# tomershay100/mp3-steganography-lib

Hardware: AMD Instinct MI355X
Metric: MP3 frames/sec (decode+re-encode) @44.1kHz stereo 128kbps, 1→8 GPU (higher is better)
Workload: dtype f64 (decode) / int32 (encode); 1 GPU; 10000-frame full decode->stego-embed->re-encode pipeline per MI355X (BASELINE configs[2]); MP3 main data + side info resident in HBM, MP3 frames out; the message cursor chain is decided and the serial chains of the rate loop are checked on the device inside every step; frames_per_gpu=10000, channels=2, message_bits=536, chain_verdict_units_to_redo=0, message_variant_entries=1874, parallelism=frames sharded over 1 GPU(s), no collective

## Files before the change

### mp3-steganography-lib_amd/csrc/k_encode.hpp

```cpp
#pragma once
#include <type_traits>
#include "analysis_plan.h"

namespace mp3s {

__device__ __forceinline__ int32_t mulhi_vs(int32_t v, int32_t s)
{
    int32_t r;
    asm("v_mul_hi_i32 %0, %1, %2" : "=v"(r) : "v"(v), "s"(s));
    return r;
}
typedef int32_t i32x4 __attribute__((ext_vector_type(4)));
typedef int32_t i32x16 __attribute__((ext_vector_type(16)));
typedef int32_t i32x8 __attribute__((ext_vector_type(8)));
template <int B, int E, class F>
__device__ __forceinline__ void static_for(F &&f)
{
    if constexpr (B < E) { f(std::integral_constant<int, B>{}); static_for<B + 1, E>(f); }
}

constexpr int ENC_ROW = 34;
constexpr int ENC_LDS_DW = 79 * 17 + 1;

constexpr int ENC_TROW = 33;
template <bool TILE, class Between>
__device__ __forceinline__ void enc_analysis_wave(const int16_t *__restrict__ pcm, const mp3s_frame_hdr *__restrict__ hdr, long Ts, int ch, long t0, int lane,
                                                  uint32_t *lds, int32_t *__restrict__ SB, uint32_t *rows, long tile_t0, long lo, long hi, Between between)
{
    int16_t *tw = reinterpret_cast<int16_t *>(lds);
    if ((reinterpret_cast<uintptr_t>(pcm) & 15u) == 0) {
        const int c0 = (int)(t0 - 15) * 8, c1 = (int)Ts * 8;
        const uint4 *gp = reinterpret_cast<const uint4 *>(pcm);
        const uint32_t sel = ch ? 0x07060302u : 0x05040100u;
        for (int c = lane; c < 79 * 8; c += 64) {
            const int gc = c0 + c;
            uint4 q = make_uint4(0, 0, 0, 0);
            if (gc >= 0 && gc < c1) q = gp[gc];
            uint2 o;
            o.x = __builtin_amdgcn_perm(q.y, q.x, sel);
            o.y = __builtin_amdgcn_perm(q.w, q.z, sel);
            uint32_t *dst = reinterpret_cast<uint32_t *>(tw + (c >> 3) * ENC_ROW + (c & 7) * 4);
            dst[0] = o.x; dst[1] = o.y;
        }
    } else {
        for (int e = lane; e < 79 * 32; e += 64) {
            const int r = e >> 5, s = e & 31;
            const long row = t0 - 15 + r;
            int16_t v = 0;
            if (row >= 0 && row < Ts) v = pcm[(row * 32 + s) * 2 + ch];
            tw[r * ENC_ROW + s] = v;
        }
    }
    __builtin_amdgcn_s_waitcnt(0xc07f);
    __builtin_amdgcn_wave_barrier();
    const long t = t0 + lane;
    const bool valid = t >= 0 && t < Ts;
    long s0 = 0;
    if (valid) s0 = (long)hdr[t / 36].stream_first * 36;

    int32_t y[64];
    const bool starts_inside = __ballot(valid && (t - 15) < s0) != 0;
    const uint32_t tw_lds = (uint32_t)(uintptr_t)(__attribute__((address_space(3))) const int16_t *)tw;
    uint32_t xs[16];
#pragma unroll
    for (int i = 0; i < 16; i++) xs[i] = 0;
#define MP3S_LDS_HI16(reg, addr, off) asm volatile("ds_read_u16_d16_hi %0, %1 offset:%2" : "+v"(reg) : "v"(addr), "n"(off))
    auto window_sums = [&](auto masked) {
    auto trip = [&](int k, auto first) {
        const i32x16 *ewa = reinterpret_cast<const i32x16 *>(c_tab.enwindow + 64 * k), *ewb = ewa + 4;
#pragma unroll
        for (int h = 0; h < 2; h++) {
            const i32x16 a0 = ewa[2 * h], a1 = ewa[2 * h + 1];
            const i32x16 b0 = ewb[2 * h], b1 = ewb[2 * h + 1];
            const int back_a = 2 * k + h, back_b = back_a + 2;
            const bool in_a = (t - back_a) >= s0, in_b = (t - back_b) >= s0;
            const uint32_t ra = tw_lds + (uint32_t)((lane + 15 - back_a) * ENC_ROW * 2), rb = ra - 2 * ENC_ROW * 2;
#pragma unroll
            for (int cb = 0; cb < 4; cb++) {
#pragma unroll
                for (int e = 0; e < 8; e++) {
                    MP3S_LDS_HI16(xs[e], ra, (cb * 8 + e) * 2);
                    MP3S_LDS_HI16(xs[8 + e], rb, (cb * 8 + e) * 2);
                }
                asm volatile("s_waitcnt lgkmcnt(0)" : "+v"(xs[0]), "+v"(xs[1]), "+v"(xs[2]), "+v"(xs[3]), "+v"(xs[4]), "+v"(xs[5]), "+v"(xs[6]), "+v"(xs[7]),
                             "+v"(xs[8]), "+v"(xs[9]), "+v"(xs[10]), "+v"(xs[11]), "+v"(xs[12]), "+v"(xs[13]), "+v"(xs[14]), "+v"(xs[15]));
#pragma unroll
                for (int e = 0; e < 8; e++) {
                    const int col = cb * 8 + e, c = 31 - col;
                    int32_t xa = (int32_t)xs[e], xb = (int32_t)xs[8 + e];
                    if (decltype(masked)::value && !in_a) xa = 0;
                    if (decltype(masked)::value && !in_b) xb = 0;
                    const int32_t two = mulhi_vs(xa, c < 16 ? a0[c & 15] : a1[c & 15]) + mulhi_vs(xb, c < 16 ? b0[c & 15] : b1[c & 15]);
                    if (decltype(first)::value) y[h * 32 + c] = two; else y[h * 32 + c] += two;
                }
                __builtin_amdgcn_sched_barrier(0);
            }
        }
    };
    trip(0, std::true_type{});
#pragma unroll 1
    for (int k = 2; k < 8; k += 2) trip(k, std::false_type{});
    };
    if (starts_inside) window_sums(std::true_type{}); else window_sums(std::false_type{});
#undef MP3S_LDS_HI16
    const bool odd_slot = (t & 1) != 0;
    __builtin_amdgcn_wave_barrier();
    between();
    uint32_t *ot = lds;
    uint32_t *out = TILE ? nullptr : reinterpret_cast<uint32_t *>(SB) + ((long)ch * Ts + t0) * 32;
    const int n_rows = (Ts - t0) < 64 ? (int)(Ts - t0) : 64;
    uint32_t *trow = TILE ? rows + (valid && t >= lo && t < hi ? (t - tile_t0) : -1) * ENC_TROW : nullptr;
    int32_t a[4] = {0, 0, 0, 0};
    i32x8 cur[4], nxt[4];
    typedef const int32_t __attribute__((address_space(4))) *fl_ptr;
    fl_ptr flp = (fl_ptr)&c_tab.fl[0][0];
    asm volatile("" : "+s"(flp));
    auto load_block = [&](auto nc, i32x8 (&c)[4]) {
        constexpr int N = decltype(nc)::value, P = N >> 3, B = N & 7;
        constexpr int O[4] = {P, 15 - P, 16 + P, 31 - P};
#pragma unroll
        for (int o = 0; o < 4; o++) c[o] = *(const i32x8 __attribute__((address_space(4))) *)(flp + O[o] * 64 + 8 * B);
    };
    load_block(std::integral_constant<int, 0>{}, cur);
    static_for<0, 64>([&](auto nc) {
        constexpr int N = decltype(nc)::value, P = N >> 3, B = N & 7;
        __builtin_amdgcn_sched_barrier(0);
        __builtin_amdgcn_s_waitcnt(0xc07f);
        __builtin_amdgcn_sched_barrier(0);
        if constexpr (N < 63) load_block(std::integral_constant<int, N + 1>{}, nxt);
        __builtin_amdgcn_sched_barrier(0);
#pragma unroll
        for (int j = 0; j < 8; j += 2) {
            int32_t m[2][4];
#pragma unroll
            for (int e = 0; e < 2; e++) {
                const int k = B * 8 + j + e;
                const unsigned plan = ANALYSIS_PLAN[P][k];
                const int32_t cj[4] = {cur[0][j + e], cur[1][j + e], cur[2][j + e], cur[3][j + e]};
#pragma unroll
                for (int o = 0; o < 4; o++) {
                    const unsigned rep = (plan >> (2 * o)) & 3u;
                    if ((plan >> (8 + o)) & 1u) m[e][o] = 0;
                    else if (rep == (unsigned)o) m[e][o] = mulhi_vs(y[k], cj[o]);
                    else m[e][o] = m[e][rep];
                }
            }
#pragma unroll
            for (int o = 0; o < 4; o++) {
                a[o] += m[0][o] + m[1][o];
                asm("" : "+v"(a[o]));
            }
            if (j == 2) __builtin_amdgcn_sched_barrier(0);
        }
        if constexpr (B == 7) {
            if (odd_slot) {
                if (P & 1) { a[0] = (int32_t)(0u - (uint32_t)a[0]); a[2] = (int32_t)(0u - (uint32_t)a[2]); }
                else       { a[1] = (int32_t)(0u - (uint32_t)a[1]); a[3] = (int32_t)(0u - (uint32_t)a[3]); }
            }
            constexpr int q = P & 3;
            if constexpr (TILE) {
                trow[P] = (uint32_t)a[0]; trow[15 - P] = (uint32_t)a[1]; trow[16 + P] = (uint32_t)a[2]; trow[31 - P] = (uint32_t)a[3];
            } else {
            ot[lane * 17 + q] = (uint32_t)a[0];
            ot[lane * 17 + 4 + 3 - q] = (uint32_t)a[1];
            ot[lane * 17 + 8 + q] = (uint32_t)a[2];
            ot[lane * 17 + 12 + 3 - q] = (uint32_t)a[3];
            }
            a[0] = a[1] = a[2] = a[3] = 0;
            if constexpr (q == 3 && !TILE) {
                constexpr int g = P >> 2;
                __builtin_amdgcn_s_waitcnt(0xc07f);
                __builtin_amdgcn_wave_barrier();
                const int piece = lane & 3;
#pragma unroll
                for (int r = lane >> 2; r < 64; r += 16) {
                    const uint32_t *src = ot + r * 17 + piece * 4;
                    const uint4 v = make_uint4(src[0], src[1], src[2], src[3]);
                    if (r < n_rows) *reinterpret_cast<uint4 *>(out + r * 32 + g * 16 + piece * 4) = v;
                }
                __builtin_amdgcn_s_waitcnt(0xc07f);
                __builtin_amdgcn_wave_barrier();
            }
        }
        if constexpr (N < 63) {
#pragma unroll
            for (int o = 0; o < 4; o++) cur[o] = nxt[o];
        }
    });
}

__device__ __forceinline__ int sb_pos(int band) { return (int)((0x37621540u >> (4 * (band >> 2))) & 7u) * 4 + (band & 3); }
__global__ __launch_bounds__(256, 5) void k_enc_analysis(
    const int16_t *__restrict__ pcm, const mp3s_frame_hdr *__restrict__ hdr, int n_frames,
    int32_t *__restrict__ SB, long Ts)
{
    __shared__ __attribute__((aligned(16))) uint32_t lds_all[4][ENC_LDS_DW];
    static_assert(79 * ENC_ROW * 2 <= ENC_LDS_DW * 4, "PCM tile must fit");
    const int wave = __builtin_amdgcn_readfirstlane(threadIdx.x >> 6), lane = threadIdx.x & 63;
    const long wid = (long)xcd_tile() * 4 + wave;
    const int ch = (int)(wid & 1);
    const long t0 = (wid >> 1) * 64;
    if (t0 >= Ts) return;
    enc_analysis_wave<false>(pcm, hdr, Ts, ch, t0, lane, lds_all[wave], SB, nullptr, 0, 0, 0, [] {});
}

constexpr int MD_ROW = 33, MD_BLK = 18 * MD_ROW;

__device__ __forceinline__ void enc_mdct_pair(const int32_t (&in)[54], int32_t *xs, int lane, int32_t *__restrict__ mdct, long ga, long g_lo, long g_hi)
{
    const int ch = lane >> 5, band = lane & 31;
    int32_t *x0 = xs + ch * MD_BLK + band, *x1 = x0 + 2 * MD_BLK;
    struct Coef { i32x4 q[9]; };
    auto load_coef = [&](int k) {
        Coef c;
        const i32x4 *crow = reinterpret_cast<const i32x4 *>(c_tab.cos_l[k]);
#pragma unroll
        for (int q = 0; q < 9; q++) c.q[q] = crow[q];
        return c;
    };
    Coef cur = load_coef(0);
#pragma unroll 2
    for (int k = 0; k < 18; k++) {
        asm volatile("" ::"s"(cur.q[0].x));
        __builtin_amdgcn_sched_barrier(0);
        const Coef nxt = load_coef(k < 17 ? k + 1 : 17);
        __builtin_amdgcn_sched_barrier(0);
        int32_t a0 = 0, a1 = 0;
#pragma unroll
        for (int q = 0; q < 9; q++) {
            const i32x4 c = cur.q[q];
            a0 += mulhi_vs(in[4 * q], c.x);     a1 += mulhi_vs(in[18 + 4 * q], c.x);
            a0 += mulhi_vs(in[4 * q + 1], c.y); a1 += mulhi_vs(in[19 + 4 * q], c.y);
            a0 += mulhi_vs(in[4 * q + 2], c.z); a1 += mulhi_vs(in[20 + 4 * q], c.z);
            a0 += mulhi_vs(in[4 * q + 3], c.w); a1 += mulhi_vs(in[21 + 4 * q], c.w);
        }
        x0[k * MD_ROW] = a0;
        x1[k * MD_ROW] = a1;
        __builtin_amdgcn_sched_barrier(0);
        cur = nxt;
    }
    __builtin_amdgcn_s_waitcnt(0xc07f);
    __builtin_amdgcn_wave_barrier();
    if (band >= 1) {
#pragma unroll
        for (int g = 0; g < 2; g++)
#pragma unroll
            for (int i = 0; i < 8; i++) {
                int32_t *pa = x0 + g * 2 * MD_BLK + i * MD_ROW, *pb = x0 + g * 2 * MD_BLK + (17 - i) * MD_ROW - 1;
                const int64_t cs = c_tab.mdct_cs[i], ca = c_tab.mdct_ca[i];
                const int64_t a = *pa, b = *pb;
                *pa = (int32_t)((a * cs - b * ca) >> 31);
                *pb = (int32_t)((a * ca + b * cs) >> 31);
            }
    }
    __builtin_amdgcn_s_waitcnt(0xc07f);
    __builtin_amdgcn_wave_barrier();
#pragma unroll
    for (int q = 0; q < 4; q++) {
        const long g = ga + (q >> 1);
        if (g < g_lo || g >= g_hi) continue;
        const int32_t *src = xs + q * MD_BLK;
        int32_t *o = mdct + (((g >> 1) * 2 + (q & 1)) * 2 + (g & 1)) * 576;
#pragma unroll
        for (int t = 0; t < 9; t++) {
            const int e = lane + 64 * t, b = (e * 3641) >> 16, k = e - 18 * b;
            o[e] = src[k * MD_ROW + b];
        }
    }
}

__global__ __launch_bounds__(256, 4) void k_enc_mdct(
    const int32_t *__restrict__ SB, long Ts, const mp3s_frame_hdr *__restrict__ hdr, int n_frames,
    int32_t *__restrict__ mdct)
{
    __shared__ int32_t xs_all[4][4 * MD_BLK];
    const int wave = __builtin_amdgcn_readfirstlane(threadIdx.x >> 6), lane = threadIdx.x & 63;
    const int f = xcd_tile() * 4 + wave;
    if (f >= n_frames) return;
    const int ch = lane >> 5, band = lane & 31;
    const bool has_prev = f > (int)hdr[f].stream_first;
    const int32_t *row = SB + ((long)ch * Ts + (long)f * 36) * 32 + sb_pos(band);
    const int32_t *prow = has_prev ? row - 18 * 32 : row;
    int32_t in[54];
#pragma unroll
    for (int j = 0; j < 18; j++) {
        const int32_t pv = prow[j * 32];
        in[j] = has_prev ? pv : 0;
        in[18 + j] = row[j * 32];
        in[36 + j] = row[(18 + j) * 32];
    }
    enc_mdct_pair(in, xs_all[wave], lane, mdct, 2l * f, 2l * f, 2l * f + 2);
}

constexpr int EF_GR = 13, EF_SLOTS = 18 * (EF_GR + 1), EF_WAVES = 8;
constexpr int EF_TILE_DW = 2 * (EF_SLOTS + 1) * ENC_TROW;
static_assert(EF_SLOTS <= 4 * 64, "four analysis waves per channel");
static_assert(EF_WAVES * ENC_LDS_DW <= EF_TILE_DW, "the waves' PCM staging fits the tile");
static_assert(((EF_GR + 1) / 2) * 4 * MD_BLK <= EF_TILE_DW, "the MDCT waves' butterfly tiles fit the tile");

__global__ __launch_bounds__(EF_WAVES * 64, 4) void k_enc_fused(
    const int16_t *__restrict__ pcm, const mp3s_frame_hdr *__restrict__ hdr, int n_frames, int32_t *__restrict__ mdct)
{
    __shared__ __attribute__((aligned(16))) uint32_t tile[EF_TILE_DW];
    const int wave = __builtin_amdgcn_readfirstlane(threadIdx.x >> 6), lane = threadIdx.x & 63;
    const long Ts = (long)n_frames * 36, n_gran = (long)n_frames * 2;
    const long g0 = (long)xcd_tile() * EF_GR;
    const long s0 = g0 * 18, t_first = s0 - 18;
    {
        const int ch = wave >> 2;
        const long t0 = t_first + 64 * (wave & 3);
        uint32_t *rows = tile + ((long)ch * (EF_SLOTS + 1) + 1) * ENC_TROW;
        enc_analysis_wave<true>(pcm, hdr, Ts, ch, t0, lane, tile + wave * ENC_LDS_DW, nullptr, rows, t_first, t_first, t_first + EF_SLOTS,
                                [] { __syncthreads(); });
    }
    __syncthreads();
    const long ga = g0 - (g0 & 1) + 2 * wave;
    const long g_hi = g0 + EF_GR < n_gran ? g0 + EF_GR : n_gran;
    const bool unit = ga < g_hi;
    int32_t in[54];
    if (unit) {
        const int ch = lane >> 5, band = lane & 31;
        const bool has_prev = ga >= g0 && ga > (long)hdr[ga >> 1].stream_first * 2;
        const long r_prev = (ga - g0) * 18;
        const uint32_t *row = tile + ((long)ch * (EF_SLOTS + 1) + 1 + (r_prev >= 0 ? r_prev : 0)) * ENC_TROW + band;
        const long r_own = r_prev >= 0 ? 18 : 0;
#pragma unroll
        for (int j = 0; j < 18; j++) {
            const int32_t pv = (int32_t)row[j * ENC_TROW];
            in[j] = has_prev ? pv : 0;
            in[18 + j] = (int32_t)row[(r_own + j) * ENC_TROW];
            in[36 + j] = ga + 1 < g_hi ? (int32_t)row[(r_own + 18 + j) * ENC_TROW] : 0;
        }
    }
    __syncthreads();
    if (unit) enc_mdct_pair(in, reinterpret_cast<int32_t *>(tile) + wave * 4 * MD_BLK, lane, mdct, ga, g0, g_hi);
}

}
```

Baseline: 19.58 million frames/s.

## Process MDCT granules sequentially to halve LDS scratch and raise occupancy

```diff
diff --git a/mp3-steganography-lib_amd/csrc/k_encode.hpp b/mp3-steganography-lib_amd/csrc/k_encode.hpp
--- a/mp3-steganography-lib_amd/csrc/k_encode.hpp
+++ b/mp3-steganography-lib_amd/csrc/k_encode.hpp
@@ -206,74 +206,85 @@
 
 constexpr int MD_ROW = 33, MD_BLK = 18 * MD_ROW;
 
+
+__device__ __forceinline__ void enc_mdct_finish(int32_t *xs, int32_t *x0, int lane, int32_t *__restrict__ mdct, long g)
+{
+    const int band = lane & 31;
+    __builtin_amdgcn_s_waitcnt(0xc07f);
+    __builtin_amdgcn_wave_barrier();
+    if (band >= 1) {
+#pragma unroll
+        for (int i = 0; i < 8; i++) {
+            int32_t *pa = x0 + i * MD_ROW, *pb = x0 + (17 - i) * MD_ROW - 1;
+            const int64_t cs = c_tab.mdct_cs[i], ca = c_tab.mdct_ca[i];
+            const int64_t a = *pa, b = *pb;
+            *pa = (int32_t)((a * cs - b * ca) >> 31);
+            *pb = (int32_t)((a * ca + b * cs) >> 31);
+        }
+    }
+    __builtin_amdgcn_s_waitcnt(0xc07f);
+    __builtin_amdgcn_wave_barrier();
+#pragma unroll
+    for (int c = 0; c < 2; c++) {
+        const int32_t *src = xs + c * MD_BLK;
+        int32_t *o = mdct + (((g >> 1) * 2 + c) * 2 + (g & 1)) * 576;
+#pragma unroll
+        for (int t = 0; t < 9; t++) {
+            const int e = lane + 64 * t, b = (e * 3641) >> 16, k = e - 18 * b;
+            o[e] = src[k * MD_ROW + b];
+        }
+    }
+    __builtin_amdgcn_s_waitcnt(0xc07f);
+    __builtin_amdgcn_wave_barrier();
+}
+
 __device__ __forceinline__ void enc_mdct_pair(const int32_t (&in)[54], int32_t *xs, int lane, int32_t *__restrict__ mdct, long ga, long g_lo, long g_hi)
 {
     const int ch = lane >> 5, band = lane & 31;
-    int32_t *x0 = xs + ch * MD_BLK + band, *x1 = x0 + 2 * MD_BLK;
+    int32_t *x0 = xs + ch * MD_BLK + band;
     struct Coef { i32x4 q[9]; };
-    auto load_coef = [&](int k) {
+    auto load_coef = [&](const int32_t (*tab)[36], int k) {
         Coef c;
-        const i32x4 *crow = reinterpret_cast<const i32x4 *>(c_tab.cos_l[k]);
+        const i32x4 *crow = reinterpret_cast<const i32x4 *>(tab[k]);
 #pragma unroll
         for (int q = 0; q < 9; q++) c.q[q] = crow[q];
         return c;
     };
-    Coef cur = load_coef(0);
+    static_for<0, 2>([&](auto gc) {
+        constexpr int g = decltype(gc)::value;
+        if (ga + g < g_lo || ga + g >= g_hi) return;
+        int z;
+        asm volatile("s_mov_b32 %0, 0" : "=s"(z));
+        const int32_t (*tab)[36] = c_tab.cos_l + z;
+        Coef cur = load_coef(tab, 0);
 #pragma unroll 2
-    for (int k = 0; k < 18; k++) {
-        asm volatile("" ::"s"(cur.q[0].x));
-        __builtin_amdgcn_sched_barrier(0);
-        const Coef nxt = load_coef(k < 17 ? k + 1 : 17);
-        __builtin_amdgcn_sched_barrier(0);
-        int32_t a0 = 0, a1 = 0;
-#pragma unroll
-        for (int q = 0; q < 9; q++) {
-            const i32x4 c = cur.q[q];
-            a0 += mulhi_vs(in[4 * q], c.x);     a1 += mulhi_vs(in[18 + 4 * q], c.x);
-            a0 += mulhi_vs(in[4 * q + 1], c.y); a1 += mulhi_vs(in[19 + 4 * q], c.y);
-            a0 += mulhi_vs(in[4 * q + 2], c.z); a1 += mulhi_vs(in[20 + 4 * q], c.z);
-            a0 += mulhi_vs(in[4 * q + 3], c.w); a1 += mulhi_vs(in[21 + 4 * q], c.w);
-        }
-        x0[k * MD_ROW] = a0;
-        x1[k * MD_ROW] = a1;
-        __builtin_amdgcn_sched_barrier(0);
-        cur = nxt;
-    }
-    __builtin_amdgcn_s_waitcnt(0xc07f);
-    __builtin_amdgcn_wave_barrier();
-    if (band >= 1) {
-#pragma unroll
-        for (int g = 0; g < 2; g++)
-#pragma unroll
-            for (int i = 0; i < 8; i++) {
-                int32_t *pa = x0 + g * 2 * MD_BLK + i * MD_ROW, *pb = x0 + g * 2 * MD_BLK + (17 - i) * MD_ROW - 1;
-                const int64_t cs = c_tab.mdct_cs[i], ca = c_tab.mdct_ca[i];
-                const int64_t a = *pa, b = *pb;
-                *pa = (int32_t)((a * cs - b * ca) >> 31);
-                *pb = (int32_t)((a * ca + b * cs) >> 31);
-            }
-    }
-    __builtin_amdgcn_s_waitcnt(0xc07f);
-    __builtin_amdgcn_wave_barrier();
-#pragma unroll
-    for (int q = 0; q < 4; q++) {
-        const long g = ga + (q >> 1);
-        if (g < g_lo || g >= g_hi) continue;
-        const int32_t *src = xs + q * MD_BLK;
-        int32_t *o = mdct + (((g >> 1) * 2 + (q & 1)) * 2 + (g & 1)) * 576;
-#pragma unroll
-        for (int t = 0; t < 9; t++) {
-            const int e = lane + 64 * t, b = (e * 3641) >> 16, k = e - 18 * b;
-            o[e] = src[k * MD_ROW + b];
-        }
-    }
-}
-
-__global__ __launch_bounds__(256, 4) void k_enc_mdct(
+        for (int k = 0; k < 18; k++) {
+            asm volatile("" ::"s"(cur.q[0].x));
+            __builtin_amdgcn_sched_barrier(0);
+            const Coef nxt = load_coef(tab, k < 17 ? k + 1 : 17);
+            __builtin_amdgcn_sched_barrier(0);
+            int32_t a = 0;
+#pragma unroll
+            for (int q = 0; q < 9; q++) {
+                const i32x4 c = cur.q[q];
+                a += mulhi_vs(in[18 * g + 4 * q], c.x);
+                a += mulhi_vs(in[18 * g + 4 * q + 1], c.y);
+                a += mulhi_vs(in[18 * g + 4 * q + 2], c.z);
+                a += mulhi_vs(in[18 * g + 4 * q + 3], c.w);
+            }
+            x0[k * MD_ROW] = a;
+            __builtin_amdgcn_sched_barrier(0);
+            cur = nxt;
+        }
+        enc_mdct_finish(xs, x0, lane, mdct, ga + g);
+    });
+}
+
+__global__ __launch_bounds__(256, 8) void k_enc_mdct(
     const int32_t *__restrict__ SB, long Ts, const mp3s_frame_hdr *__restrict__ hdr, int n_frames,
     int32_t *__restrict__ mdct)
 {
-    __shared__ int32_t xs_all[4][4 * MD_BLK];
+    __shared__ int32_t xs_all[4][2 * MD_BLK];
     const int wave = __builtin_amdgcn_readfirstlane(threadIdx.x >> 6), lane = threadIdx.x & 63;
     const int f = xcd_tile() * 4 + wave;
     if (f >= n_frames) return;
@@ -286,9 +297,11 @@
     for (int j = 0; j < 18; j++) {
         const int32_t pv = prow[j * 32];
         in[j] = has_prev ? pv : 0;
-        in[18 + j] = row[j * 32];
-        in[36 + j] = row[(18 + j) * 32];
-    }
+    }
+#pragma unroll
+    for (int j = 0; j < 18; j++) in[18 + j] = row[j * 32];
+#pragma unroll
+    for (int j = 0; j < 18; j++) in[36 + j] = row[(18 + j) * 32];
     enc_mdct_pair(in, xs_all[wave], lane, mdct, 2l * f, 2l * f, 2l * f + 2);
 }
 
@@ -296,7 +309,7 @@
 constexpr int EF_TILE_DW = 2 * (EF_SLOTS + 1) * ENC_TROW;
 static_assert(EF_SLOTS <= 4 * 64, "four analysis waves per channel");
 static_assert(EF_WAVES * ENC_LDS_DW <= EF_TILE_DW, "the waves' PCM staging fits the tile");
-static_assert(((EF_GR + 1) / 2) * 4 * MD_BLK <= EF_TILE_DW, "the MDCT waves' butterfly tiles fit the tile");
+static_assert(((EF_GR + 1) / 2) * 2 * MD_BLK <= EF_TILE_DW, "the MDCT waves' butterfly tiles fit the tile");
 
 __global__ __launch_bounds__(EF_WAVES * 64, 4) void k_enc_fused(
     const int16_t *__restrict__ pcm, const mp3s_frame_hdr *__restrict__ hdr, int n_frames, int32_t *__restrict__ mdct)
@@ -333,7 +346,7 @@
         }
     }
     __syncthreads();
-    if (unit) enc_mdct_pair(in, reinterpret_cast<int32_t *>(tile) + wave * 4 * MD_BLK, lane, mdct, ga, g0, g_hi);
-}
-
-}
+    if (unit) enc_mdct_pair(in, reinterpret_cast<int32_t *>(tile) + wave * 2 * MD_BLK, lane, mdct, ga, g0, g_hi);
+}
+
+}
```

New measurement: 19.53 million frames/s. Within noise of the previous version (-0.2%).
